# zhiqwang/demonet

Hardware: AMD Instinct MI355X
Metric: images/sec ssdlite320_mobilenet_v3_large fp16 end-to-end incl. NMS (higher is better)
Workload: dtype fp16; 1 GPU; ssdlite320_mobilenet_v3_large fp16, batch 64 per GPU, 320x320 synthetic images, K=91, synthetic weights seed 0, post-process incl. per-class top-300 + hard NMS; global_batch=64, forwards_in_flight=3, parallelism=single GPU, input=NCHW fp32 in [0,1], device-resident

## Files before the change

demonet_amd/_lib.py:

```python
import ctypes as C
import os

_HERE = os.path.dirname(os.path.abspath(__file__))
LIB_PATH = os.environ.get("DEMONET_HIP_LIB") or os.path.join(_HERE, "lib", "libdemonet_hip.so")
DN_ABI_VERSION = 1

DN_OP = dict(stem=1, pw=2, dw=3, se=4, conv=5, maxpool=6, l2norm=7)
DN_T = dict(act=0, image=1, vec=2, pool=3)
DN_NMS = dict(hard=0, linear=1, gaussian=2)
DN_MERGE = dict(iou=0, ios=1)
DN_SGD_CHUNK = 2048
DN_SGD_MAX_GATE = 8


class TensorDesc(C.Structure):
    _fields_ = [("c", C.c_int32), ("h", C.c_int32), ("w", C.c_int32), ("kind", C.c_int32)]


class OpDesc(C.Structure):
    _fields_ = [("type", C.c_int32), ("inp", C.c_int32), ("out", C.c_int32), ("residual", C.c_int32),
                ("se", C.c_int32), ("pool", C.c_int32),
                ("cin", C.c_int32), ("cout", C.c_int32), ("k", C.c_int32), ("stride", C.c_int32), ("pad", C.c_int32),
                ("dil", C.c_int32), ("act", C.c_int32),
                ("head", C.c_int32), ("level", C.c_int32), ("squeeze", C.c_int32), ("ceil_mode", C.c_int32),
                ("pool_pixels", C.c_int32), ("reserved", C.c_int32 * 2),
                ("w_off", C.c_int64), ("b_off", C.c_int64), ("w2_off", C.c_int64), ("b2_off", C.c_int64)]


class SgdTensor(C.Structure):
    _fields_ = [("p", C.c_void_p), ("g", C.c_void_p), ("buf", C.c_void_p), ("numel", C.c_int64)]


class SgdHyper(C.Structure):
    _fields_ = [("lr", C.c_float), ("momentum", C.c_float), ("dampening", C.c_float), ("weight_decay", C.c_float),
                ("nesterov", C.c_int32), ("first_step", C.c_int32), ("step", C.c_int32), ("reserved", C.c_int32)]


class ModelDesc(C.Structure):
    _fields_ = [("abi_version", C.c_int32), ("n_tensors", C.c_int32), ("n_ops", C.c_int32),
                ("tensors", C.POINTER(TensorDesc)), ("ops", C.POINTER(OpDesc)),
                ("input_tensor", C.c_int32), ("image_h", C.c_int32), ("image_w", C.c_int32),
                ("mean", C.c_float * 3), ("std", C.c_float * 3),
                ("num_classes", C.c_int32), ("n_levels", C.c_int32),
                ("level_tensor", C.c_int32 * 8), ("anchors_per_loc", C.c_int32 * 8),
                ("num_anchors", C.c_int32), ("anchors", C.POINTER(C.c_float)),
                ("score_thresh", C.c_float), ("nms_thresh", C.c_float),
                ("detections_per_img", C.c_int32), ("topk_candidates", C.c_int32)]


_SIGNATURES = {
    "dn_abi_version": (C.c_int, []),
    "dn_last_error": (C.c_char_p, []),
    "dn_create": (C.c_int, [C.POINTER(ModelDesc), C.c_void_p, C.c_size_t, C.POINTER(C.c_void_p)]),
    "dn_destroy": (None, [C.c_void_p]),
    "dn_workspace_bytes": (C.c_size_t, [C.c_void_p, C.c_int]),
    "dn_forward": (C.c_int, [C.c_void_p, C.c_void_p, C.c_int, C.c_int, C.c_int, C.c_void_p, C.c_void_p, C.c_void_p,
                             C.c_void_p, C.c_void_p, C.c_size_t, C.c_void_p]),
    "dn_forward_u8": (C.c_int, [C.c_void_p, C.c_void_p, C.c_int, C.c_int, C.c_int, C.c_void_p, C.c_void_p, C.c_void_p,
                             C.c_void_p, C.c_void_p, C.c_size_t, C.c_void_p]),
    "dn_forward_heads": (C.c_int, [C.c_void_p, C.c_void_p, C.c_int, C.c_int, C.c_int, C.c_void_p, C.c_size_t, C.c_void_p]),
    "dn_head_outputs": (C.c_int, [C.c_void_p, C.c_void_p, C.c_int, C.POINTER(C.c_void_p), C.POINTER(C.c_void_p)]),
    "dn_tensor_ptr": (C.c_int, [C.c_void_p, C.c_void_p, C.c_int, C.c_int, C.POINTER(C.c_void_p), C.POINTER(C.c_size_t)]),
    "dn_postprocess_workspace_bytes": (C.c_size_t, [C.c_int, C.c_int, C.c_int, C.c_int, C.c_int]),
    "dn_postprocess": (C.c_int, [C.c_void_p, C.c_void_p, C.c_void_p, C.c_int, C.c_int, C.c_int, C.c_float, C.c_float,
                                 C.c_void_p, C.c_float, C.c_float, C.c_int, C.c_int, C.c_void_p, C.c_void_p, C.c_void_p,
                                 C.c_void_p, C.c_void_p, C.c_void_p, C.c_size_t, C.c_void_p]),
    "dn_postprocess_soft": (C.c_int, [C.c_void_p, C.c_void_p, C.c_void_p, C.c_int, C.c_int, C.c_int, C.c_float, C.c_float,
                                      C.c_void_p, C.c_float, C.c_float, C.c_int, C.c_float, C.c_int, C.c_int, C.c_void_p, C.c_void_p, C.c_void_p,
                                      C.c_void_p, C.c_void_p, C.c_void_p, C.c_size_t, C.c_void_p]),
    "dn_set_nms": (C.c_int, [C.c_void_p, C.c_int, C.c_float]),
    "dn_pointwise_conv": (C.c_int, [C.c_void_p, C.c_void_p, C.c_void_p, C.c_void_p, C.c_void_p, C.c_void_p, C.c_void_p, C.c_int,
                                    C.c_int, C.c_int, C.c_int, C.c_int, C.c_int, C.c_int64, C.c_void_p]),
    "dn_depthwise_conv": (C.c_int, [C.c_void_p, C.c_void_p, C.c_void_p, C.c_void_p, C.c_int, C.c_int, C.c_int, C.c_int,
                                    C.c_int, C.c_int, C.c_int, C.c_int, C.c_void_p]),
    "dn_dense_conv": (C.c_int, [C.c_void_p] * 5 + [C.c_int] * 10 + [C.c_void_p]),
    "dn_expand_depthwise": (C.c_int, [C.c_void_p] * 9 + [C.c_int] * 11 + [C.c_void_p]),
    "dn_expand_depthwise_tiles": (C.c_int, [C.c_int, C.c_int, C.c_int]),
    "dn_ssd_loss_workspace_bytes": (C.c_size_t, [C.c_int, C.c_int]),
    "dn_ssd_loss": (C.c_int, [C.c_void_p] * 6 + [C.c_int] * 4 + [C.c_float, C.c_float] + [C.c_void_p, C.c_void_p, C.c_void_p, C.c_size_t, C.c_void_p]),
    "dn_ssd_loss_state_bytes": (C.c_size_t, [C.c_int, C.c_int]),
    "dn_ssd_loss_train": (C.c_int, [C.c_void_p] * 6 + [C.c_int] * 4 + [C.c_float, C.c_float] + [C.c_void_p, C.c_void_p, C.c_void_p, C.c_size_t, C.c_void_p, C.c_size_t,
                                    C.c_void_p]),
    "dn_ssd_loss_backward": (C.c_int, [C.c_void_p] * 6 + [C.c_size_t, C.c_void_p] + [C.c_int] * 4 + [C.c_void_p] * 3),
    "dn_set_graph_mode": (C.c_int, [C.c_void_p, C.c_int]),
    "dn_set_packed_output": (C.c_int, [C.c_void_p, C.c_void_p]),
    "dn_profile_begin": (C.c_int, [C.c_void_p]),
    "dn_profile_end": (C.c_int, [C.c_void_p, C.POINTER(C.c_float), C.c_int]),
    "dn_batch_split": (C.c_int, [C.c_void_p, C.c_int]),
    "dn_set_chains": (C.c_int, [C.c_void_p, C.c_int]),
    "dn_profile_op_info": (C.c_int, [C.c_void_p, C.c_int, C.c_char_p, C.c_int, C.POINTER(C.c_int32)]),
    "dn_level_features": (C.c_int, [C.c_void_p, C.c_void_p, C.c_int, C.c_int, C.c_int, C.POINTER(C.c_void_p), C.POINTER(C.c_int), C.POINTER(C.c_int)]),
    "dn_forward_features": (C.c_int, [C.c_void_p, C.c_void_p, C.c_int, C.c_int, C.c_int, C.c_void_p, C.c_size_t, C.c_void_p]),
    "dn_lite_head_backward_workspace_bytes": (C.c_size_t, [C.c_int] * 6),
    "dn_lite_head_backward": (C.c_int, [C.c_void_p] * 5 + [C.c_int64] + [C.c_int] * 5 + [C.c_void_p] * 5 + [C.c_size_t, C.c_void_p]),
    "dn_crop_tiles": (C.c_int, [C.c_void_p, C.c_int, C.c_int, C.c_void_p, C.c_int, C.c_int, C.c_int, C.c_void_p, C.c_void_p]),
    "dn_merge_detections_workspace_bytes": (C.c_size_t, [C.c_int] * 3),
    "dn_merge_detections": (C.c_int, [C.c_void_p] * 5 + [C.c_int, C.c_int, C.POINTER(C.c_int32), C.c_int, C.c_int, C.c_float, C.c_int, C.c_int] + [C.c_void_p] * 6
                            + [C.c_size_t, C.c_void_p]),
    "dn_fuse_detections_workspace_bytes": (C.c_size_t, [C.c_int, C.c_int, C.POINTER(C.c_int32), C.c_int]),
    "dn_fuse_detections": (C.c_int, [C.c_void_p] * 6 + [C.c_int, C.c_int, C.POINTER(C.c_int32), C.c_int, C.c_float, C.c_float, C.c_int] + [C.c_void_p] * 6
                           + [C.c_size_t, C.c_void_p]),
    "dn_match_detections": (C.c_int, [C.c_void_p] * 8 + [C.c_int] * 4 + [C.POINTER(C.c_double), C.c_int, C.c_double] + [C.c_void_p] * 5),
    "dn_coco_match": (C.c_int, [C.c_void_p] * 9 + [C.c_int] * 4 + [C.POINTER(C.c_double), C.c_int, C.POINTER(C.c_double), C.c_int, C.c_int] + [C.c_void_p] * 5),
    "dn_augment_workspace_bytes": (C.c_size_t, [C.c_int]),
    "dn_augment_batch": (C.c_int, [C.POINTER(C.c_void_p), C.POINTER(C.c_int32), C.POINTER(C.c_int32), C.c_int, C.c_int, C.c_int, C.c_void_p, C.c_void_p, C.c_size_t, C.c_void_p]),
    "dn_sgd_workspace_bytes": (C.c_size_t, [C.c_int, C.c_int]),
    "dn_grad_norm": (C.c_int, [C.c_void_p, C.c_int, C.c_int, C.c_void_p, C.c_size_t, C.c_void_p, C.c_void_p]),
    "dn_sgd_step": (C.c_int, [C.c_void_p, C.c_int, C.c_int, SgdHyper, C.c_void_p, C.c_int, C.c_void_p, C.c_float, C.c_void_p, C.c_void_p]),
}
EXPORTS = tuple(_SIGNATURES)

_lib = None


class HipLibraryMissing(RuntimeError):
    pass


def lib():
    global _lib
    if _lib is not None:
        return _lib
    if not os.path.exists(LIB_PATH):
        raise HipLibraryMissing(
            f"{LIB_PATH} not found: build it with `python -m demonet_amd.build` (hipcc, gfx950). "
            "demonet_amd has no CPU fallback.")
    L = C.CDLL(LIB_PATH)
    for name, (res, args) in _SIGNATURES.items():
        fn = getattr(L, name)
        fn.restype = res
        fn.argtypes = args
    if L.dn_abi_version() != DN_ABI_VERSION:
        raise HipLibraryMissing(f"ABI mismatch: library {L.dn_abi_version()} vs binding {DN_ABI_VERSION}; rebuild")
    _lib = L
    return L


def check(rc: int, what: str = ""):
    if rc < 0:
        msg = lib().dn_last_error().decode("utf-8", "replace")
        raise RuntimeError(f"demonet_hip {what} failed ({rc}): {msg}")
    return rc
```

demonet_amd/csrc/depthwise.hip:

```cpp
#include "choice.h"

#ifdef DN_DEV_STAMPS
static long long* g_se_stamps = nullptr;
extern "C" __attribute__((visibility("default"))) void dn_debug_se_stamps(void* dev_ptr) { g_se_stamps = (long long*)dev_ptr; }
#else
constexpr long long* g_se_stamps = nullptr;
#endif

namespace {

__device__ const uint4 g_dw_zero16 = {0u, 0u, 0u, 0u};

__device__ __forceinline__ void dw_se_tail(const DwArgs& a, const int n, const int nblk, float* sh) {
    const int c = a.c, sq = a.se_sq, tid = threadIdx.x;
    float* mean = sh;
    float* z = sh + c;
    float* part = z + sq;
    {
        const float* p0 = a.pool + (size_t)n * nblk * c;
        for (int ic = tid; ic < c; ic += 256) {
            float t = 0.f;
            for (int b0 = 0; b0 < nblk; b0 += 16) {
                float v[16];
#pragma unroll
                for (int u = 0; u < 16; ++u) v[u] = __hip_atomic_load(&p0[(size_t)min(b0 + u, nblk - 1) * c + ic], __ATOMIC_RELAXED, __HIP_MEMORY_SCOPE_AGENT);
#pragma unroll
                for (int u = 0; u < 16; ++u) t += (b0 + u < nblk) ? v[u] : 0.f;
            }
            mean[ic] = t * a.se_inv;
        }
    }
    __syncthreads();
    auto fc = [&](const half_t* wt, const float* bias, const float* in, int nin, int nout, float* out, bool hsig) {
        const int OG = (nout + 7) >> 3;
        int ogp = 1;
        while (ogp < OG) ogp <<= 1;
        const int KS = 256 / ogp;
        const int og = tid & (ogp - 1), ks = tid / ogp;
        const int per = (nin + KS - 1) / KS, i0 = ks * per, i1 = min(nin, i0 + per);
        float acc[8] = {0, 0, 0, 0, 0, 0, 0, 0};
        if (og < OG && i0 < i1) {
            const half_t* wp = wt + (size_t)og * 8;
            for (int ib = i0; ib < i1; ib += 16) {
                uint4 v[16];
#pragma unroll
                for (int u = 0; u < 16; ++u) v[u] = *reinterpret_cast<const uint4*>(wp + (size_t)min(ib + u, i1 - 1) * nout);
#pragma unroll
                for (int u = 0; u < 16; ++u) {
                    const float m = (ib + u < i1) ? in[ib + u] : 0.f;
                    const half8 h = *reinterpret_cast<const half8*>(&v[u]);
#pragma unroll
                    for (int e = 0; e < 8; ++e) acc[e] += (float)h[e] * m;
                }
            }
        }
#pragma unroll
        for (int e = 0; e < 8; ++e) part[tid * 8 + e] = acc[e];
        __syncthreads();
        for (int j = tid; j < nout; j += 256) {
            float t = bias[j];
            const int g = j >> 3, e = j & 7;
            for (int q = 0; q < KS; ++q) t += part[(q * ogp + g) * 8 + e];
            out[j] = hsig ? fminf(fmaxf(t + 3.f, 0.f), 6.f) * (1.f / 6.f) : fmaxf(t, 0.f);
        }
        __syncthreads();
    };
    fc(a.se_w1t, a.se_b1, mean, c, sq, z, false);
    fc(a.se_w2t, a.se_b2, z, sq, c, a.se_scale + (size_t)n * c, true);
}

__device__ __forceinline__ void dw_se_tail_small(const DwArgs& a, const int n, const int nblk, float* sh) {
    const int c = a.c, sq = a.se_sq, tid = threadIdx.x;
    float* mean = sh;
    float* z = sh + c;
    float* part = z + sq;
    const int OG1 = (sq + 7) >> 3, OG2 = (c + 7) >> 3;
    int ogp1 = 1, ogp2 = 1;
    while (ogp1 < OG1) ogp1 <<= 1;
    while (ogp2 < OG2) ogp2 <<= 1;
    const int KS1 = 256 / ogp1, KS2 = 256 / ogp2;
    const int og1 = tid & (ogp1 - 1), ks1 = tid / ogp1, per1 = (c + KS1 - 1) / KS1, i0 = ks1 * per1, i1 = min(c, i0 + per1);
    const int og2 = tid & (ogp2 - 1), ks2 = tid / ogp2, per2 = (sq + KS2 - 1) / KS2, j0 = ks2 * per2, j1 = min(sq, j0 + per2);
    const bool act1 = og1 < OG1 && i0 < i1, act2 = og2 < OG2 && j0 < j1;
    float pv[32];
    {
        const float* p0 = a.pool + (size_t)n * nblk * c + min(tid, c - 1);
#pragma unroll
        for (int b = 0; b < 32; ++b) pv[b] = __hip_atomic_load(&p0[(size_t)min(b, nblk - 1) * c], __ATOMIC_RELAXED, __HIP_MEMORY_SCOPE_AGENT);
    }
    uint4 w1[2], w2[2];
#pragma unroll
    for (int u = 0; u < 2; ++u) {
        w1[u] = *reinterpret_cast<const uint4*>(a.se_w1t + (size_t)min(i0 + u, c - 1) * sq + min(og1, OG1 - 1) * 8);
        w2[u] = *reinterpret_cast<const uint4*>(a.se_w2t + (size_t)min(j0 + u, sq - 1) * c + min(og2, OG2 - 1) * 8);
    }
    const float b1v = a.se_b1[min(tid, sq - 1)], b2v = a.se_b2[min(tid, c - 1)];
    if (tid < c) {
        float t = 0.f;
#pragma unroll
        for (int b = 0; b < 32; ++b) t += (b < nblk) ? pv[b] : 0.f;
        mean[tid] = t * a.se_inv;
    }
    __syncthreads();
    auto fc = [&](const uint4 (&w)[2], bool act, int r0, int r1, const float* in, int ogp, int KS, int nout, float bias, float* out, bool hsig) {
        float acc[8] = {0, 0, 0, 0, 0, 0, 0, 0};
        if (act) {
#pragma unroll
            for (int u = 0; u < 2; ++u) {
                const float m = (r0 + u < r1) ? in[r0 + u] : 0.f;
                const half8 h = *reinterpret_cast<const half8*>(&w[u]);
#pragma unroll
                for (int e = 0; e < 8; ++e) acc[e] += (float)h[e] * m;
            }
        }
#pragma unroll
        for (int e = 0; e < 8; ++e) part[tid * 8 + e] = acc[e];
        __syncthreads();
        if (tid < nout) {
            float t = bias;
            const int g = tid >> 3, e = tid & 7;
            for (int q = 0; q < KS; ++q) t += part[(q * ogp + g) * 8 + e];
            out[tid] = hsig ? fminf(fmaxf(t + 3.f, 0.f), 6.f) * (1.f / 6.f) : fmaxf(t, 0.f);
        }
        __syncthreads();
    };
    fc(w1, act1, i0, i1, mean, ogp1, KS1, sq, b1v, z, false);
    fc(w2, act2, j0, j1, z, ogp2, KS2, c, b2v, a.se_scale + (size_t)n * c, true);
}
__device__ __forceinline__ bool dw_se_tail_is_small(int c, int sq, int nblk) {
    if (!(se_is_small(c, sq) && nblk <= 32)) return false;
    int ogp1 = 1, ogp2 = 1;
    while (ogp1 < ((sq + 7) >> 3)) ogp1 <<= 1;
    while (ogp2 < ((c + 7) >> 3)) ogp2 <<= 1;
    const int ks1 = 256 / ogp1, ks2 = 256 / ogp2;
    return (c + ks1 - 1) / ks1 <= 2 && (sq + ks2 - 1) / ks2 <= 2;
}

template <int K, int S, int TW, int POOL>
__device__ __forceinline__ void dw_body(const DwArgs& a, const int bx, const int nblocks, const int n) {
    constexpr int NIN = (TW - 1) * S + K;
    extern __shared__ float red[];
    const unsigned C8 = a.c >> 3;
    const unsigned idx0 = bx * 256 + threadIdx.x;
    const unsigned q1 = fd_div(idx0, a.fd_c8);
    const unsigned cg = idx0 - q1 * C8;
    const unsigned oy = fd_div(q1, a.fd_xs);
    const unsigned xs = q1 - oy * a.fd_xs.d;
    const bool valid = (int)oy < a.ho;
    if (!valid && POOL == 0) return;
    const int ox0 = xs * TW;
    const unsigned c0 = cg * 8;
    float psum[8] = {0, 0, 0, 0, 0, 0, 0, 0};
    if (valid) {

    float acc[TW][8];
    {
        const float4 b0 = *reinterpret_cast<const float4*>(a.bias + c0);
        const float4 b1 = *reinterpret_cast<const float4*>(a.bias + c0 + 4);
#pragma unroll
        for (int t = 0; t < TW; ++t) {
            acc[t][0] = b0.x; acc[t][1] = b0.y; acc[t][2] = b0.z; acc[t][3] = b0.w;
            acc[t][4] = b1.x; acc[t][5] = b1.y; acc[t][6] = b1.z; acc[t][7] = b1.w;
        }
    }
    const int ix0 = ox0 * S - a.pad;
    typedef const __attribute__((address_space(1))) half8* gp8;
    const gp8 zero = (gp8)(&g_dw_zero16);
    const half_t* const wbase = a.w + c0;
    const half_t* const xbase = a.x + (size_t)n * a.h * a.w_ * a.c + c0;
    half8 wv[2][K];
    half8 xin[2][NIN];
    auto load_row = [&](const int ky, const int buf) {
        const int iy = (int)oy * S - a.pad + ky;
        const bool yok = iy >= 0 && iy < a.h;
#pragma unroll
        for (int kx = 0; kx < K; ++kx) wv[buf][kx] = *reinterpret_cast<const half8*>(wbase + (unsigned)((ky * K + kx) * a.c));
        const half_t* rowp = xbase + (unsigned)((yok ? iy : 0) * a.w_ * a.c);
#pragma unroll
        for (int i = 0; i < NIN; ++i) {
            const int ix = ix0 + i;
            const bool ok = yok && ix >= 0 && ix < a.w_;
            xin[buf][i] = *(ok ? (gp8)(rowp + (unsigned)(ix * a.c)) : zero);
        }
    };
    load_row(0, 0);
#pragma unroll
    for (int ky = 0; ky < K; ++ky) {
        if (ky + 1 < K) load_row(ky + 1, (ky + 1) & 1);
#pragma unroll
        for (int t = 0; t < TW; ++t)
#pragma unroll
            for (int kx = 0; kx < K; ++kx)
                fma_mix_h8(acc[t], *reinterpret_cast<const uint4*>(&xin[ky & 1][t * S + kx]), *reinterpret_cast<const uint4*>(&wv[ky & 1][kx]));
    }
    half_t* orow = a.out + ((size_t)(n * a.ho + oy) * a.wo) * a.c + c0;
#pragma unroll
    for (int t = 0; t < TW; ++t) {
        if (ox0 + t >= a.wo) break;
        dn_act_n<float[8], 8>(acc[t], a.act);
        half8 o;
#pragma unroll
        for (int e = 0; e < 8; ++e) {
            if constexpr (POOL != 0) psum[e] += acc[t][e];
            o[e] = (half_t)acc[t][e];
        }
        *reinterpret_cast<half8*>(orow + (unsigned)((ox0 + t) * a.c)) = o;
    }
    }
    if constexpr (POOL != 0) {
#pragma unroll
        for (int e = 0; e < 8; ++e) red[threadIdx.x * 8 + e] = psum[e];
        __syncthreads();
        if (threadIdx.x < C8) {
            const unsigned i1 = bx * 256 + threadIdx.x;
            const unsigned cgp = i1 - fd_div(i1, a.fd_c8) * C8;
            float t8[8] = {0, 0, 0, 0, 0, 0, 0, 0};
            for (unsigned u = threadIdx.x; u < 256; u += C8)
#pragma unroll
                for (int e = 0; e < 8; ++e) t8[e] += red[u * 8 + e];
            float* dst = a.pool + ((size_t)n * nblocks + bx) * a.c + cgp * 8;
            if constexpr (POOL == 2) {
#pragma unroll
                for (int e = 0; e < 8; ++e) __hip_atomic_store(&dst[e], t8[e], __ATOMIC_RELAXED, __HIP_MEMORY_SCOPE_AGENT);
                asm volatile("s_waitcnt vmcnt(0)" ::: "memory");
            } else {
#pragma unroll
                for (int e = 0; e < 8; ++e) dst[e] = t8[e];
            }
        }
        if constexpr (POOL == 2) {
            __shared__ int s_last;
            __syncthreads();
            if (threadIdx.x == 0)
                s_last = __hip_atomic_fetch_add(&a.se_counter[n], 1u, __ATOMIC_RELAXED, __HIP_MEMORY_SCOPE_AGENT) == (unsigned)(nblocks - 1);
            __syncthreads();
            if (s_last) {
                if (dw_se_tail_is_small(a.c, a.se_sq, nblocks)) dw_se_tail_small(a, n, nblocks, red);
                else dw_se_tail(a, n, nblocks, red);
                if (threadIdx.x == 0) a.se_counter[n] = 0u;
            }
        }
    }
}

template <int K, int S, int TW, int POOL>
__global__ __launch_bounds__(256) __attribute__((amdgpu_waves_per_eu(K == 3 ? 4 : 3))) void dw_kernel(DwArgs a, int nblocks) {
    int img, bx;
    if (!xcd_image_of2(a.xq, a.n, img, bx)) return;
    dw_body<K, S, TW, POOL>(a, bx, nblocks, img);
}

struct DwGroup {
    int count;
    int start[13];
    int nblocks[12];
    DwArgs a[12];
};

template <int K, int S, int TW>
__global__ __launch_bounds__(256) __attribute__((amdgpu_waves_per_eu(K == 3 ? 4 : 1))) void dw_group_kernel(DwGroup g) {
    int p = 0;
#pragma unroll
    for (int i = 1; i < 12; ++i)
        if (i < g.count && (int)blockIdx.x >= g.start[i]) p = i;
    const DwArgs& a = g.a[p];
    const int rel = blockIdx.x - g.start[p];
    int img, bx;
    if (a.xq > 0) { img = (rel & 7) * a.xq + blockIdx.y; bx = rel >> 3; }
    else { img = blockIdx.y; bx = rel; }
    if (img >= a.n) return;
    dw_body<K, S, TW, 0>(a, bx, g.nblocks[p], img);
}

bool dw_fill(DwArgs& a, const int tw) {
    const unsigned c8 = a.c / 8, xs = (a.wo + tw - 1) / tw;
    a.fd_c8 = fastdiv(c8);
    a.fd_xs = fastdiv(xs);
    const unsigned long long threads = (unsigned long long)a.ho * xs * c8 + 256;
    return fd_ok(threads, c8) && fd_ok(threads / c8 + 1, xs) && (unsigned long long)a.h * a.w_ * a.c < 0x80000000ull;
}
int dw_blocks(const DwArgs& a, const int tw) { return dn_cdiv((long)a.ho * ((a.wo + tw - 1) / tw) * (a.c / 8), 256); }

template <int K_, int S_>
struct DwInst { static constexpr int K = K_, S = S_, TW = dw_tw(S_); };
template <class F>
int dw_dispatch(const DwChoice& c, F&& f) {
    if (c.k == 3 && c.stride == 1) return f(DwInst<3, 1>{});
    if (c.k == 3 && c.stride == 2) return f(DwInst<3, 2>{});
    if (c.k == 5 && c.stride == 1) return f(DwInst<5, 1>{});
    if (c.k == 5 && c.stride == 2) return f(DwInst<5, 2>{});
    dn_set_error("depthwise: unsupported k=%d stride=%d", c.k, c.stride);
    return DN_E_UNSUPPORTED;
}

template <int K, int S, int TW>
int launch_dw_group(const DwArgs* arr, int count, hipStream_t s) {
    DwGroup g{};
    g.count = count;
    int acc = 0;
    for (int i = 0; i < count; ++i) {
        g.a[i] = arr[i];
        DN_REQUIRE(dw_fill(g.a[i], TW), "depthwise group: problem %d outside the index range of the kernel", i);
        g.start[i] = acc;
        g.nblocks[i] = dw_blocks(arr[i], TW);
        acc += g.nblocks[i] * (arr[i].xq > 0 ? 8 : 1);
    }
    g.start[count] = acc;
    dn_note_kernel("dw_group_kernel<%d,%d,%d>", K, S, TW);
    hipLaunchKernelGGL((dw_group_kernel<K, S, TW>), dim3(acc, arr[0].xq > 0 ? arr[0].xq : arr[0].n), dim3(256), 0, s, g);
    return DN_OK;
}

template <int K, int S, int TW>
int launch_dw(const DwArgs& a0, const DwChoice::Pool pool, hipStream_t s) {
    DwArgs a = a0;
    DN_REQUIRE(dw_fill(a, TW), "depthwise: %d x %d x %d outside the index range of the kernel", a.ho, a.wo, a.c);
    dn_note_kernel("dw_kernel<%d,%d,%d>", K, S, TW);
    const int nblocks = dw_blocks(a, TW);
    const dim3 grid = xcd_grid2(nblocks, a.xq, a.n);
    switch (pool) {
        case DwChoice::NO_POOL: hipLaunchKernelGGL((dw_kernel<K, S, TW, 0>), grid, dim3(256), 0, s, a, nblocks); break;
        case DwChoice::POOLED: hipLaunchKernelGGL((dw_kernel<K, S, TW, 1>), grid, dim3(256), (size_t)256 * 8 * 4, s, a, nblocks); break;
        case DwChoice::POOLED_SE:
            DN_REQUIRE(a.pool && a.se_counter && depthwise_se_tail_supported(a.c, a.se_sq), "depthwise: squeeze-excitation tail needs the pooled output and c <= 1024, squeeze <= 256, both multiples of 8");
            hipLaunchKernelGGL((dw_kernel<K, S, TW, 2>), grid, dim3(256), (size_t)(a.c + a.se_sq + 2048) * 4, s, a, nblocks);
            break;
    }
    return DN_OK;
}

__global__ __launch_bounds__(1024) void se_fc_kernel(const float* __restrict__ partial, int nblk, const unsigned* __restrict__ w1t,
                                                   const float* __restrict__ b1, const unsigned* __restrict__ w2t,
                                                   const float* __restrict__ b2, float* __restrict__ scale,
                                                   int c, int sq, float inv_pixels, long long* __restrict__ stamps, int nimg, int xq) {
#ifdef DN_DEV_STAMPS
#define SE_STAMP(k) do { if (stamps && threadIdx.x == 0) stamps[blockIdx.x * 8 + (k)] = (long long)__builtin_amdgcn_s_memrealtime(); } while (0)
#else
#define SE_STAMP(k) do { } while (0)
#endif
    extern __shared__ float sh[];
    float* mean = sh;
    float* z = sh + c;
    float* part = z + sq;
    int n, unused;
    if (!xcd_image_of(blockIdx.x, 1, xq, nimg, n, unused)) return;
    const int tid = threadIdx.x;
    SE_STAMP(0);
    const int sq2 = sq >> 1, c2 = c >> 1;
    const int JP = sq2;
    const int KS1 = 1024 / JP;
    const int j = tid % JP, r1 = tid / JP;
    const int per1 = (c + KS1 - 1) / KS1;
    const int i0 = r1 * per1, i1 = min(c, i0 + per1);
    const bool act1 = j < sq2 && r1 < KS1;
    const int CP = c2;
    const int KS2 = max(1, 1024 / CP);
    const int i = tid % CP, r2 = tid / CP;
    const int per2 = (sq + KS2 - 1) / KS2;
    const int j0 = r2 * per2, j1 = min(sq, j0 + per2);
    const bool act2 = i < c2 && r2 < KS2;
    constexpr int FB = 32;
    {
        const int CPm = (c + 63) & ~63;
        const int RS = max(1, min(1024 / CPm, nblk));
        const int ic = tid % CPm, r = tid / CPm;
        float t = 0.f;
        if (ic < c && r < RS) {
            const float* p = partial + (size_t)n * nblk * c + ic;
            for (int b0 = r; b0 < nblk; b0 += RS * 16) {
                float v[16];
#pragma unroll
                for (int u = 0; u < 16; ++u) v[u] = p[(size_t)min(b0 + u * RS, nblk - 1) * c];
#pragma unroll
                for (int u = 0; u < 16; ++u) t += (b0 + u * RS < nblk) ? v[u] : 0.f;
            }
        }
        part[tid] = t;
        __syncthreads();
        if (tid < c) {
            float m = 0.f;
            for (int q = 0; q < RS; ++q) m += part[q * CPm + tid];
            mean[tid] = m * inv_pixels;
        }
        __syncthreads();
    }
    SE_STAMP(1);
    auto lo = [](unsigned w) { return (float)__builtin_bit_cast(half_t, (unsigned short)(w & 0xffffu)); };
    auto hi = [](unsigned w) { return (float)__builtin_bit_cast(half_t, (unsigned short)(w >> 16)); };
    {
        float t0 = 0.f, t1 = 0.f;
        if (act1) {
            for (int ib = i0; ib < i1; ib += FB) {
                unsigned v[FB];
#pragma unroll
                for (int u = 0; u < FB; ++u) v[u] = w1t[(size_t)min(ib + u, i1 - 1) * sq2 + j];
#pragma unroll
                for (int u = 0; u < FB; ++u) {
                    const float m = (ib + u < i1) ? mean[ib + u] : 0.f;
                    t0 += lo(v[u]) * m;
                    t1 += hi(v[u]) * m;
                }
            }
        }
        part[tid] = t0;
        part[1024 + tid] = t1;
        __syncthreads();
        if (tid < sq) {
            float a = b1[tid];
// ... 773 lines not shown
```

demonet_amd/csrc/plan.hip:

```cpp
#include <stdarg.h>
#include <stdlib.h>
#include <string.h>

#include <algorithm>
#include <cmath>
#include <atomic>
#include <map>
#include <mutex>
#include <set>
#include <string>
#include <tuple>
#include <vector>

#include "choice.h"

static thread_local char g_err[512] = "";

static thread_local char g_kernel[96] = "";
void dn_note_kernel(const char* fmt, ...) {
    va_list ap;
    va_start(ap, fmt);
    vsnprintf(g_kernel, sizeof(g_kernel), fmt, ap);
    va_end(ap);
}
// ... 1342 lines not shown
    return launch_postprocess(a, reinterpret_cast<hipStream_t>(stream), nullptr);
}

extern "C" int dn_postprocess(const float* logits, const float* reg, const float* anchors, int n, int A, int K, float image_h,
                              float image_w, const float* scale_xy, float score_thresh, float nms_thresh, int topk, int dets,
                              float* boxes, float* scores, int64_t* labels, int32_t* counts, int32_t* kept_anchor, void* ws,
                              size_t ws_bytes, void* stream) {
    return dn_postprocess_soft(logits, reg, anchors, n, A, K, image_h, image_w, scale_xy, score_thresh, nms_thresh, DN_NMS_HARD, 0.f, topk, dets,
                               boxes, scores, labels, counts, kept_anchor, ws, ws_bytes, stream);
}

extern "C" int dn_pointwise_conv(const void* x, const void* w, const void* w_frag, const float* bias, const void* residual,
                                 const float* se, void* out, int m, int cin, int cout, int hw, int act, int out_fp32,
                                 int64_t out_img_stride, void* stream) {
    DN_REQUIRE(x && w && bias && out, "dn_pointwise_conv: null argument");
    PwArgs a;
    a.x = reinterpret_cast<const half_t*>(x); a.w = reinterpret_cast<const half_t*>(w); a.bias = bias;
    a.wfrag = reinterpret_cast<const half_t*>(w_frag);
    a.residual = reinterpret_cast<const half_t*>(residual); a.se = se; a.out = out;
    a.m = m; a.cin = cin; a.cout = cout; a.hw = hw; a.act = act; a.out_fp32 = out_fp32;
    a.out_img_stride = out_fp32 ? (long)out_img_stride : 0; a.out_base = 0;
    a.xq = (hw > 0 && m % hw == 0) ? xcd_images_per_group(m / hw) : 0;
    int rc = launch_pointwise(a, reinterpret_cast<hipStream_t>(stream));
    if (rc) return rc;
    DN_HIP_CHECK(hipGetLastError());
    return DN_OK;
}

extern "C" int dn_expand_depthwise(const void* x, const void* w1, const float* b1, const void* wd, const float* bd, const void* w3,
                                   const float* b3, void* out, float* pool_partial, int n, int h, int w, int cin, int cexp, int cout,
                                   int k, int stride, int act1, int act2, int has_res, void* stream) {
    DN_REQUIRE(x && wd && bd && out, "dn_expand_depthwise: null argument");
    DN_REQUIRE((w1 == nullptr) == (b1 == nullptr) && (w3 == nullptr) == (b3 == nullptr), "dn_expand_depthwise: weight without bias");
    ExpDwArgs a{};
    a.x = reinterpret_cast<const half_t*>(x); a.out = reinterpret_cast<half_t*>(out); a.pool = pool_partial;
    a.w1 = reinterpret_cast<const half_t*>(w1); a.b1 = b1; a.wd = reinterpret_cast<const half_t*>(wd); a.bd = bd;
    a.w3 = reinterpret_cast<const half_t*>(w3); a.b3 = b3;
    a.n = n; a.H = h; a.W = w; a.k = k; a.stride = stride; a.pad = (k - 1) / 2;
    a.Ho = (h + 2 * a.pad - k) / stride + 1; a.Wo = (w + 2 * a.pad - k) / stride + 1;
    a.cin = cin; a.cexp = cexp; a.cout = w3 ? cout : cexp; a.act1 = act1; a.act2 = act2; a.has_res = has_res;
    a.xq = xcd_images_per_group(n);
    int rc = launch_expdw(a, reinterpret_cast<hipStream_t>(stream));
    if (rc) return rc;
    DN_HIP_CHECK(hipGetLastError());
    return DN_OK;
}

extern "C" int dn_expand_depthwise_tiles(int ho, int wo, int stride) { return expdw_tiles_per_image(ho, wo, stride); }

extern "C" int dn_dense_conv(const void* x, const void* w, const float* bias, const void* zeros, void* out, int n, int h, int wd,
                             int cin, int cout, int k, int stride, int pad, int dil, int act, void* stream) {
    DN_REQUIRE(x && w && bias && out, "dn_dense_conv: null argument");
    DN_REQUIRE(n > 0 && h > 0 && wd > 0 && k >= 1 && stride >= 1 && dil >= 1 && pad >= 0, "dn_dense_conv: bad geometry");
    ConvArgs a;
    a.x = reinterpret_cast<const half_t*>(x); a.w = reinterpret_cast<const half_t*>(w); a.bias = bias; a.out = out;
    a.zeros = reinterpret_cast<const half_t*>(zeros);
    a.n = n; a.h = h; a.w_ = wd; a.cin = cin; a.cout = cout; a.k = k; a.stride = stride; a.pad = pad; a.dil = dil; a.act = act;
    a.ho = (h + 2 * pad - dil * (k - 1) - 1) / stride + 1;
    a.wo = (wd + 2 * pad - dil * (k - 1) - 1) / stride + 1;
    DN_REQUIRE(a.ho > 0 && a.wo > 0, "dn_dense_conv: empty output");
    a.out_fp32 = 0; a.out_img_stride = 0; a.out_base = 0;
    a.xq = xcd_images_per_group(n);
    int rc = launch_conv(a, reinterpret_cast<hipStream_t>(stream));
    if (rc) return rc;
    DN_HIP_CHECK(hipGetLastError());
    return DN_OK;
}

extern "C" int dn_depthwise_conv(const void* x, const void* w, const float* bias, void* out, int n, int h, int wd, int c, int k,
                                 int stride, int pad, int act, void* stream) {
    DN_REQUIRE(x && w && bias && out, "dn_depthwise_conv: null argument");
    DwArgs a;
    a.x = reinterpret_cast<const half_t*>(x); a.w = reinterpret_cast<const half_t*>(w); a.bias = bias;
    a.out = reinterpret_cast<half_t*>(out);
    a.n = n; a.h = h; a.w_ = wd; a.c = c; a.k = k; a.stride = stride; a.pad = pad; a.act = act;
    a.ho = (h + 2 * pad - k) / stride + 1;
    a.wo = (wd + 2 * pad - k) / stride + 1;
    a.xq = xcd_images_per_group(n);
    int rc = launch_depthwise(a, reinterpret_cast<hipStream_t>(stream));
    if (rc) return rc;
    DN_HIP_CHECK(hipGetLastError());
    return DN_OK;
}
```

include/demonet_hip.h:

```cpp
#ifndef DEMONET_HIP_H
#define DEMONET_HIP_H

#include <stddef.h>
#include <stdint.h>

#ifdef __cplusplus
extern "C" {
#endif

#define DN_ABI_VERSION 1
#define DN_MAX_CLASSES 2048
#define DN_API __attribute__((visibility("default")))

enum { DN_OK = 0, DN_E_INVALID = -1, DN_E_HIP = -2, DN_E_WORKSPACE = -3, DN_E_UNSUPPORTED = -4 };

enum { DN_ACT_NONE = 0, DN_ACT_RELU = 1, DN_ACT_RELU6 = 2, DN_ACT_HSWISH = 3 };

enum { DN_OP_STEM = 1, DN_OP_PW = 2, DN_OP_DW = 3, DN_OP_SE = 4, DN_OP_CONV = 5, DN_OP_MAXPOOL = 6, DN_OP_L2NORM = 7 };

enum { DN_T_ACT = 0, DN_T_IMAGE = 1, DN_T_VEC = 2, DN_T_POOL = 3 };

typedef struct dn_tensor_desc {
    int32_t c, h, w, kind;
} dn_tensor_desc;

typedef struct dn_op_desc {
    int32_t type;
    int32_t in, out;
    int32_t residual;
    int32_t se;
    int32_t pool;
    int32_t cin, cout, k, stride, pad, dil, act;
    int32_t head;
    int32_t level;
    int32_t squeeze;
    int32_t ceil_mode;
    int32_t pool_pixels;
    int32_t reserved[2];
    int64_t w_off, b_off, w2_off, b2_off;
} dn_op_desc;

typedef struct dn_model_desc {
    int32_t abi_version;
    int32_t n_tensors, n_ops;
    const dn_tensor_desc* tensors;
    const dn_op_desc* ops;
    int32_t input_tensor;
    int32_t image_h, image_w;
    float mean[3], std[3];
    int32_t num_classes;
    int32_t n_levels;
    int32_t level_tensor[8];
    int32_t anchors_per_loc[8];
    int32_t num_anchors;
    const float* anchors;
    float score_thresh, nms_thresh;
    int32_t detections_per_img, topk_candidates;
} dn_model_desc;

typedef struct dn_plan dn_plan;

DN_API int dn_create(const dn_model_desc* desc, const void* weights, size_t weight_bytes, dn_plan** out);
DN_API void dn_destroy(dn_plan* plan);

DN_API size_t dn_workspace_bytes(const dn_plan* plan, int n);

DN_API int dn_forward(dn_plan* plan, const float* images_dev, int n, int h, int w,
               float* boxes_dev, float* scores_dev, int64_t* labels_dev, int32_t* counts_dev,
               void* workspace_dev, size_t workspace_bytes, void* stream);

DN_API int dn_forward_u8(dn_plan* plan, const uint8_t* images_dev, int n, int h, int w,
                  float* boxes_dev, float* scores_dev, int64_t* labels_dev, int32_t* counts_dev,
                  void* workspace_dev, size_t workspace_bytes, void* stream);

DN_API int dn_forward_heads(dn_plan* plan, const float* images_dev, int n, int h, int w,
                     void* workspace_dev, size_t workspace_bytes, void* stream);
DN_API int dn_head_outputs(const dn_plan* plan, void* workspace_dev, int n, float** cls_logits_dev, float** bbox_regression_dev);
DN_API int dn_tensor_ptr(const dn_plan* plan, void* workspace_dev, int n, int tensor_id, void** ptr, size_t* bytes);

DN_API int dn_level_features(const dn_plan* plan, void* workspace_dev, int n, int level, int chain, void** ptr, int* first_image, int* images);
DN_API int dn_forward_features(dn_plan* plan, const float* images_dev, int n, int h, int w,
                               void* workspace_dev, size_t workspace_bytes, void* stream);

DN_API size_t dn_postprocess_workspace_bytes(int n, int num_anchors, int num_classes, int topk_candidates, int detections_per_img);
DN_API int dn_postprocess(const float* cls_logits_dev, const float* bbox_regression_dev, const float* anchors_dev,
                   int n, int num_anchors, int num_classes,
                   float image_h, float image_w, const float* scale_xy_dev ,
                   float score_thresh, float nms_thresh, int topk_candidates, int detections_per_img,
                   float* boxes_dev, float* scores_dev, int64_t* labels_dev, int32_t* counts_dev,
                   int32_t* kept_anchor_dev, void* workspace_dev, size_t workspace_bytes, void* stream);

enum { DN_NMS_HARD = 0, DN_NMS_SOFT_LINEAR = 1, DN_NMS_SOFT_GAUSSIAN = 2 };
DN_API int dn_set_nms(dn_plan* plan, int method, float sigma);
DN_API int dn_postprocess_soft(const float* cls_logits_dev, const float* bbox_regression_dev, const float* anchors_dev,
                   int n, int num_anchors, int num_classes,
                   float image_h, float image_w, const float* scale_xy_dev ,
                   float score_thresh, float nms_thresh, int nms_method, float nms_sigma, int topk_candidates, int detections_per_img,
                   float* boxes_dev, float* scores_dev, int64_t* labels_dev, int32_t* counts_dev,
                   int32_t* kept_anchor_dev, void* workspace_dev, size_t workspace_bytes, void* stream);

DN_API int dn_pointwise_conv(const void* x_dev, const void* w_dev, const void* w_frag_dev, const float* bias_dev,
                      const void* residual_dev, const float* se_scale_dev, void* out_dev, int m, int cin, int cout, int hw,
                      int act, int out_fp32, int64_t out_img_stride, void* stream);
DN_API int dn_dense_conv(const void* x_dev, const void* w_dev, const float* bias_dev, const void* zeros_dev, void* out_dev,
                  int n, int h, int w, int cin, int cout, int k, int stride, int pad, int dil, int act, void* stream);
DN_API int dn_depthwise_conv(const void* x_dev, const void* w_dev, const float* bias_dev, void* out_dev,
                      int n, int h, int w, int c, int k, int stride, int pad, int act, void* stream);

DN_API int dn_expand_depthwise(const void* x_dev, const void* w1_dev, const float* b1_dev, const void* wd_dev, const float* bd_dev,
                        const void* w3_dev, const float* b3_dev, void* out_dev, float* pool_partial_dev,
                        int n, int h, int w, int cin, int cexp, int cout, int k, int stride, int act1, int act2, int has_res,
                        void* stream);
DN_API int dn_expand_depthwise_tiles(int ho, int wo, int stride);

DN_API int dn_set_graph_mode(dn_plan* plan, int enabled);

DN_API int dn_profile_begin(dn_plan* plan);
DN_API int dn_profile_end(dn_plan* plan, float* ms_per_op , int capacity);
DN_API int dn_profile_op_info(const dn_plan* plan, int op_index, char* kernel, int capacity, int32_t* owner);

DN_API int dn_set_packed_output(dn_plan* plan, float* packed_dev);

DN_API int dn_batch_split(const dn_plan* plan, int n);
DN_API int dn_set_chains(dn_plan* plan, int chains);

DN_API size_t dn_ssd_loss_workspace_bytes(int n, int num_anchors);
DN_API int dn_ssd_loss(const float* cls_logits_dev, const float* bbox_regression_dev, const float* anchors_dev,
                       const float* gt_boxes_dev, const int64_t* gt_labels_dev, const int32_t* gt_counts_dev,
                       int n, int num_anchors, int num_classes, int gmax, float iou_thresh, float neg_to_pos_ratio,
                       int64_t* matched_idxs_dev, float* losses_dev, void* workspace_dev, size_t workspace_bytes, void* stream);

DN_API size_t dn_ssd_loss_state_bytes(int n, int num_anchors);
DN_API int dn_ssd_loss_train(const float* cls_logits_dev, const float* bbox_regression_dev, const float* anchors_dev,
                             const float* gt_boxes_dev, const int64_t* gt_labels_dev, const int32_t* gt_counts_dev,
                             int n, int num_anchors, int num_classes, int gmax, float iou_thresh, float neg_to_pos_ratio,
                             int64_t* matched_idxs_dev, float* losses_dev, void* workspace_dev, size_t workspace_bytes,
                             void* state_dev, size_t state_bytes, void* stream);
DN_API int dn_ssd_loss_backward(const float* cls_logits_dev, const float* bbox_regression_dev, const float* anchors_dev,
                                const float* gt_boxes_dev, const int64_t* gt_labels_dev, const void* state_dev, size_t state_bytes,
                                const float* grad_losses_dev, int n, int num_anchors, int num_classes, int gmax,
                                float* grad_cls_logits_dev, float* grad_bbox_regression_dev, void* stream);

DN_API size_t dn_lite_head_backward_workspace_bytes(int n, int h, int w, int c, int cout, int depthwise);
DN_API int dn_lite_head_backward(const void* x_dev, const void* wd_dev, const float* bd_dev, const void* w1_dev, const float* dy_dev,
                                 int64_t dy_img_stride, int n, int h, int w, int c, int cout, float* g_wd_dev, float* g_bd_dev,
                                 float* g_w1_dev, float* g_b1_dev, void* workspace_dev, size_t workspace_bytes, void* stream);

DN_API int dn_crop_tiles(const float* image_dev, int h, int w, const int32_t* origins_dev, int t, int th, int tw, float* out_dev, void* stream);

enum { DN_MERGE_IOU = 0, DN_MERGE_IOS = 1 };
DN_API size_t dn_merge_detections_workspace_bytes(int s_total, int d, int groups);
DN_API int dn_merge_detections(const float* boxes_dev, const float* scores_dev, const int64_t* labels_dev, const int32_t* counts_dev,
                               const float* offsets_dev, int s_total, int d, const int32_t* group_begin, int groups, int metric, float thresh,
                               int class_agnostic, int d_out, float* boxes_out_dev, float* scores_out_dev, int64_t* labels_out_dev,
                               int32_t* counts_out_dev, int32_t* src_out_dev, void* workspace_dev, size_t workspace_bytes, void* stream);

DN_API size_t dn_fuse_detections_workspace_bytes(int s_total, int d, const int32_t* group_begin, int groups);
DN_API int dn_fuse_detections(const float* boxes_dev, const float* scores_dev, const int64_t* labels_dev, const int32_t* counts_dev,
                              const float* offsets_dev, const float* weights_dev, int s_total, int d, const int32_t* group_begin, int groups,
                              float thresh, float skip_thresh, int d_out, float* boxes_out_dev, float* scores_out_dev, int64_t* labels_out_dev,
                              int32_t* counts_out_dev, int32_t* members_out_dev, void* workspace_dev, size_t workspace_bytes, void* stream);

DN_API int dn_match_detections(const float* boxes_dev, const float* scores_dev, const int64_t* labels_dev, const int32_t* counts_dev,
                               const float* gt_boxes_dev, const int64_t* gt_labels_dev, const uint8_t* gt_difficult_dev,
                               const int32_t* gt_counts_dev, int n, int d, int gmax, int num_classes, const double* thresholds, int n_thresh,
                               double pixel_offset, uint32_t* flags_dev, int32_t* best_gt_dev, double* best_ov_dev, int64_t* gt_stats_dev,
                               void* stream);

DN_API int dn_coco_match(const float* boxes_dev, const float* scores_dev, const int64_t* labels_dev, const int32_t* counts_dev,
                         const float* gt_boxes_dev, const int64_t* gt_labels_dev, const int32_t* gt_counts_dev, const uint8_t* gt_crowd_dev,
                         const float* gt_area_dev, int n, int d, int gmax, int num_classes, const double* thresholds, int n_thresh,
                         const double* area_ranges, int n_ranges, int max_det, uint32_t* flags_dev, int32_t* rank_dev, int32_t* match_gt_dev,
                         int64_t* gt_stats_dev, void* stream);

enum { DN_AUG_FLAGS = 0,
       DN_AUG_BRIGHTNESS = 1, DN_AUG_CONTRAST = 2, DN_AUG_SATURATION = 3, DN_AUG_HUE = 4,
       DN_AUG_PERM = 5,
       DN_AUG_CANVAS_H = 8, DN_AUG_CANVAS_W = 9, DN_AUG_LEFT = 10, DN_AUG_TOP = 11,
       DN_AUG_FILL = 12,
       DN_AUG_CROP_L = 15, DN_AUG_CROP_T = 16, DN_AUG_CROP_W = 17, DN_AUG_CROP_H = 18,
       DN_AUG_WORDS = 20 };
enum { DN_AUG_F_BRIGHTNESS = 1, DN_AUG_F_CONTRAST = 2, DN_AUG_F_SATURATION = 4, DN_AUG_F_HUE = 8, DN_AUG_F_CONTRAST_BEFORE = 16, DN_AUG_F_FLIP = 32,
       DN_AUG_F_ALL = 63 };
DN_API size_t dn_augment_workspace_bytes(int n);
DN_API int dn_augment_batch(const uint8_t* const* images, const int32_t* sizes, const int32_t* params, int n, int out_h, int out_w,
                            float* out_dev, void* workspace_dev, size_t workspace_bytes, void* stream);

#define DN_SGD_CHUNK 2048
#define DN_SGD_MAX_GATE 8
typedef struct dn_sgd_tensor {
// ... 24 lines not shown
```

Baseline: 107,300 images/sec.

## Stage depthwise weights and bias in LDS and use buffer loads for inputs

For depthwise convolutions with at most 128 channels, each block now copies the filter taps (transposed so each channel group's taps are contiguous) and the bias into shared memory, then reads weights from LDS instead of global memory. Input rows are fetched with raw buffer loads whose out-of-range offsets return zero, replacing the pointer select to a zero constant. The first input row is prefetched before the weight staging to overlap the two. It also adds a pooled depthwise API entry point and debug timestamp hooks. The cost is extra shared memory per block and a block-wide barrier, which may reduce occupancy; the waves-per-EU hint is raised for this path.

```diff
diff --git a/demonet_amd/_lib.py b/demonet_amd/_lib.py
--- a/demonet_amd/_lib.py
+++ b/demonet_amd/_lib.py
@@ -73,6 +73,8 @@
                                     C.c_int, C.c_int, C.c_int, C.c_int, C.c_int, C.c_int64, C.c_void_p]),
     "dn_depthwise_conv": (C.c_int, [C.c_void_p, C.c_void_p, C.c_void_p, C.c_void_p, C.c_int, C.c_int, C.c_int, C.c_int,
                                     C.c_int, C.c_int, C.c_int, C.c_int, C.c_void_p]),
+    "dn_depthwise_pool_blocks": (C.c_int, [C.c_int] * 6),
+    "dn_depthwise_conv_pool": (C.c_int, [C.c_void_p] * 4 + [C.c_int] * 8 + [C.c_void_p] * 7 + [C.c_int, C.c_void_p]),
     "dn_dense_conv": (C.c_int, [C.c_void_p] * 5 + [C.c_int] * 10 + [C.c_void_p]),
     "dn_expand_depthwise": (C.c_int, [C.c_void_p] * 9 + [C.c_int] * 11 + [C.c_void_p]),
     "dn_expand_depthwise_tiles": (C.c_int, [C.c_int, C.c_int, C.c_int]),
diff --git a/demonet_amd/csrc/depthwise.hip b/demonet_amd/csrc/depthwise.hip
--- a/demonet_amd/csrc/depthwise.hip
+++ b/demonet_amd/csrc/depthwise.hip
@@ -3,8 +3,16 @@
 #ifdef DN_DEV_STAMPS
 static long long* g_se_stamps = nullptr;
 extern "C" __attribute__((visibility("default"))) void dn_debug_se_stamps(void* dev_ptr) { g_se_stamps = (long long*)dev_ptr; }
+static long long* g_dw_stamps = nullptr;
+extern "C" __attribute__((visibility("default"))) void dn_debug_dw_stamps(void* dev_ptr) { g_dw_stamps = (long long*)dev_ptr; }
+#define DW_STAMPS_PARAM , long long* const stamps
+#define DW_STAMPS_ARG(p) , p
+#define DW_STAMP(k) do { if (stamps && threadIdx.x == 0) stamps[((size_t)n * nblocks + bx) * 8 + (k)] = (long long)__builtin_amdgcn_s_memrealtime(); } while (0)
 #else
 constexpr long long* g_se_stamps = nullptr;
+#define DW_STAMPS_PARAM
+#define DW_STAMPS_ARG(p)
+#define DW_STAMP(k) do { } while (0)
 #endif
 
 namespace {
@@ -136,10 +144,12 @@
     return (c + ks1 - 1) / ks1 <= 2 && (sq + ks2 - 1) / ks2 <= 2;
 }
 
-template <int K, int S, int TW, int POOL>
-__device__ __forceinline__ void dw_body(const DwArgs& a, const int bx, const int nblocks, const int n) {
-    constexpr int NIN = (TW - 1) * S + K;
-    extern __shared__ float red[];
+template <int K, int S, int TW, int POOL, bool WLDS>
+__device__ __forceinline__ void dw_body(const DwArgs& a, const int bx, const int nblocks, const int n DW_STAMPS_PARAM) {
+    constexpr int NIN = (TW - 1) * S + K, KK = K * K;
+    extern __shared__ __attribute__((aligned(16))) float dw_sh[];
+    float* const red = WLDS ? dw_sh + (KK * a.c) / 2 + a.c : dw_sh;
+    DW_STAMP(0);
     const unsigned C8 = a.c >> 3;
     const unsigned idx0 = bx * 256 + threadIdx.x;
     const unsigned q1 = fd_div(idx0, a.fd_c8);
@@ -147,30 +157,66 @@
     const unsigned oy = fd_div(q1, a.fd_xs);
     const unsigned xs = q1 - oy * a.fd_xs.d;
     const bool valid = (int)oy < a.ho;
-    if (!valid && POOL == 0) return;
+    if (!valid && POOL == 0 && !WLDS) return;
     const int ox0 = xs * TW;
     const unsigned c0 = cg * 8;
+    const int ix0 = ox0 * S - a.pad;
     float psum[8] = {0, 0, 0, 0, 0, 0, 0, 0};
+    half8 xin[2][NIN];
+    const unsigned c2 = (unsigned)a.c * 2u;
+    const __amdgpu_buffer_rsrc_t xrs = __builtin_amdgcn_make_buffer_rsrc(const_cast<half_t*>(a.x + (size_t)n * a.h * a.w_ * a.c), 0, WLDS ? a.h * a.w_ * a.c * 2 : 0, 0x00020000);
+    auto load_row_buf = [&](const int ky, const int buf) {
+        const int iy = (int)oy * S - a.pad + ky;
+        const bool yok = valid && (unsigned)iy < (unsigned)a.h;
+        const unsigned rowoff = (unsigned)((iy * a.w_ + ix0) * a.c + (int)c0) * 2u;
+#pragma unroll
+        for (int i = 0; i < NIN; ++i) {
+            const bool ok = yok && (unsigned)(ix0 + i) < (unsigned)a.w_;
+            xin[buf][i] = __builtin_bit_cast(half8, __builtin_amdgcn_raw_buffer_load_b128(xrs, ok ? rowoff + (unsigned)i * c2 : 0x80000000u, 0, 0));
+        }
+    };
+    if constexpr (WLDS) {
+        load_row_buf(0, 0);
+        const uint4* const wsrc = reinterpret_cast<const uint4*>(a.w);
+        uint4* const wdst = reinterpret_cast<uint4*>(dw_sh);
+        const unsigned nitems = KK * C8;
+        const unsigned one = a.fd_c8.d == 1 ? ~0u : 0u;
+        float4* const bdst = reinterpret_cast<float4*>(dw_sh + (KK * a.c) / 2);
+        const unsigned bi = min(threadIdx.x, ((unsigned)a.c >> 2) - 1);
+        const float4 bv = reinterpret_cast<const float4*>(a.bias)[bi];
+        for (unsigned i0 = threadIdx.x; i0 < nitems; i0 += 1024) {
+            uint4 v[4];
+#pragma unroll
+            for (int u = 0; u < 4; ++u) v[u] = wsrc[min(i0 + u * 256, nitems - 1)];
+#pragma unroll
+            for (int u = 0; u < 4; ++u) {
+                const unsigned i = min(i0 + u * 256, nitems - 1), tap = __umulhi(i, a.fd_c8.m) + (i & one);
+                wdst[(i - tap * C8) * KK + tap] = v[u];
+            }
+        }
+        bdst[bi] = bv;
+        __syncthreads();
+    }
+    DW_STAMP(1);
     if (valid) {
 
     float acc[TW][8];
     {
-        const float4 b0 = *reinterpret_cast<const float4*>(a.bias + c0);
-        const float4 b1 = *reinterpret_cast<const float4*>(a.bias + c0 + 4);
+        const float* const bsrc = WLDS ? dw_sh + (KK * a.c) / 2 : a.bias;
+        const float4 b0 = *reinterpret_cast<const float4*>(bsrc + c0);
+        const float4 b1 = *reinterpret_cast<const float4*>(bsrc + c0 + 4);
 #pragma unroll
         for (int t = 0; t < TW; ++t) {
             acc[t][0] = b0.x; acc[t][1] = b0.y; acc[t][2] = b0.z; acc[t][3] = b0.w;
             acc[t][4] = b1.x; acc[t][5] = b1.y; acc[t][6] = b1.z; acc[t][7] = b1.w;
         }
     }
-    const int ix0 = ox0 * S - a.pad;
     typedef const __attribute__((address_space(1))) half8* gp8;
     const gp8 zero = (gp8)(&g_dw_zero16);
     const half_t* const wbase = a.w + c0;
     const half_t* const xbase = a.x + (size_t)n * a.h * a.w_ * a.c + c0;
     half8 wv[2][K];
-    half8 xin[2][NIN];
-    auto load_row = [&](const int ky, const int buf) {
+    auto load_row_ptr = [&](const int ky, const int buf) {
         const int iy = (int)oy * S - a.pad + ky;
         const bool yok = iy >= 0 && iy < a.h;
 #pragma unroll
@@ -183,20 +229,42 @@
             xin[buf][i] = *(ok ? (gp8)(rowp + (unsigned)(ix * a.c)) : zero);
         }
     };
-    load_row(0, 0);
+    auto load_row = [&](const int ky, const int buf) {
+        if constexpr (WLDS) load_row_buf(ky, buf);
+        else load_row_ptr(ky, buf);
+    };
+    const uint4* const wl = reinterpret_cast<const uint4*>(dw_sh) + cg * KK;
+    if constexpr (!WLDS) load_row(0, 0);
 #pragma unroll
     for (int ky = 0; ky < K; ++ky) {
         if (ky + 1 < K) load_row(ky + 1, (ky + 1) & 1);
-#pragma unroll
-        for (int t = 0; t < TW; ++t)
-#pragma unroll
-            for (int kx = 0; kx < K; ++kx)
-                fma_mix_h8(acc[t], *reinterpret_cast<const uint4*>(&xin[ky & 1][t * S + kx]), *reinterpret_cast<const uint4*>(&wv[ky & 1][kx]));
-    }
+        if constexpr (WLDS) {
+#pragma unroll
+            for (int kx = 0; kx < K; ++kx) {
+                const uint4 w = wl[ky * K + kx];
+#pragma unroll
+                for (int t = 0; t < TW; ++t) fma_mix_h8(acc[t], *reinterpret_cast<const uint4*>(&xin[ky & 1][t * S + kx]), w);
+            }
+        } else {
+#pragma unroll
+            for (int t = 0; t < TW; ++t)
+#pragma unroll
+                for (int kx = 0; kx < K; ++kx)
+                    fma_mix_h8(acc[t], *reinterpret_cast<const uint4*>(&xin[ky & 1][t * S + kx]), *reinterpret_cast<const uint4*>(&wv[ky & 1][kx]));
+        }
+    }
+    DW_STAMP(2);
     half_t* orow = a.out + ((size_t)(n * a.ho + oy) * a.wo) * a.c + c0;
+    int ox0s = ox0;
+    if constexpr (POOL != 0 && !WLDS) {
+        unsigned t2 = threadIdx.x;
+        asm volatile("" : "+v"(t2));
+        const unsigned q2 = fd_div(bx * 256 + t2, a.fd_c8);
+        ox0s = (int)(q2 - fd_div(q2, a.fd_xs) * a.fd_xs.d) * TW;
+    }
 #pragma unroll
     for (int t = 0; t < TW; ++t) {
-        if (ox0 + t >= a.wo) break;
+        if (ox0s + t >= a.wo) break;
         dn_act_n<float[8], 8>(acc[t], a.act);
         half8 o;
 #pragma unroll
@@ -204,9 +272,10 @@
             if constexpr (POOL != 0) psum[e] += acc[t][e];
             o[e] = (half_t)acc[t][e];
         }
-        *reinterpret_cast<half8*>(orow + (unsigned)((ox0 + t) * a.c)) = o;
-    }
-    }
+        *reinterpret_cast<half8*>(orow + (unsigned)((ox0s + t) * a.c)) = o;
+    }
+    }
+    DW_STAMP(3);
     if constexpr (POOL != 0) {
 #pragma unroll
         for (int e = 0; e < 8; ++e) red[threadIdx.x * 8 + e] = psum[e];
@@ -230,24 +299,27 @@
         }
         if constexpr (POOL == 2) {
             __shared__ int s_last;
+            DW_STAMP(4);
             __syncthreads();
             if (threadIdx.x == 0)
                 s_last = __hip_atomic_fetch_add(&a.se_counter[n], 1u, __ATOMIC_RELAXED, __HIP_MEMORY_SCOPE_AGENT) == (unsigned)(nblocks - 1);
             __syncthreads();
+            DW_STAMP(5);
             if (s_last) {
-                if (dw_se_tail_is_small(a.c, a.se_sq, nblocks)) dw_se_tail_small(a, n, nblocks, red);
-                else dw_se_tail(a, n, nblocks, red);
+                if (dw_se_tail_is_small(a.c, a.se_sq, nblocks)) dw_se_tail_small(a, n, nblocks, dw_sh);
+                else dw_se_tail(a, n, nblocks, dw_sh);
                 if (threadIdx.x == 0) a.se_counter[n] = 0u;
-            }
-        }
-    }
-}
-
-template <int K, int S, int TW, int POOL>
-__global__ __launch_bounds__(256) __attribute__((amdgpu_waves_per_eu(K == 3 ? 4 : 3))) void dw_kernel(DwArgs a, int nblocks) {
+                DW_STAMP(6);
+            }
+        }
+    }
+}
+
+template <int K, int S, int TW, int POOL, bool WLDS>
+__global__ __launch_bounds__(256) __attribute__((amdgpu_waves_per_eu(K == 3 || WLDS ? 4 : 3))) void dw_kernel(DwArgs a, int nblocks DW_STAMPS_PARAM) {
     int img, bx;
     if (!xcd_image_of2(a.xq, a.n, img, bx)) return;
-    dw_body<K, S, TW, POOL>(a, bx, nblocks, img);
+    dw_body<K, S, TW, POOL, WLDS>(a, bx, nblocks, img DW_STAMPS_ARG(stamps));
 }
 
 struct DwGroup {
@@ -269,7 +341,7 @@
     if (a.xq > 0) { img = (rel & 7) * a.xq + blockIdx.y; bx = rel >> 3; }
     else { img = blockIdx.y; bx = rel; }
     if (img >= a.n) return;
-    dw_body<K, S, TW, 0>(a, bx, g.nblocks[p], img);
+    dw_body<K, S, TW, 0, false>(a, bx, g.nblocks[p], img DW_STAMPS_ARG(nullptr));
 }
 
 bool dw_fill(DwArgs& a, const int tw) {
@@ -280,6 +352,14 @@
     return fd_ok(threads, c8) && fd_ok(threads / c8 + 1, xs) && (unsigned long long)a.h * a.w_ * a.c < 0x80000000ull;
 }
 int dw_blocks(const DwArgs& a, const int tw) { return dn_cdiv((long)a.ho * ((a.wo + tw - 1) / tw) * (a.c / 8), 256); }
+
+size_t dw_wlds_bytes(const DwArgs& a, const int k) {
+    const int knob = dn_knob("DN_DW_WLDS", 1);
+    if (knob == 0 || (knob != 2 && a.c > 128)) return 0;
+    const size_t bytes = (size_t)k * k * a.c * 2 + (size_t)a.c * 4;
+    const bool ok = a.c <= 1024 && bytes + 256 * 8 * 4 <= 64 * 1024 && (unsigned long long)a.h * a.w_ * a.c < 0x40000000ull && fd_ok((unsigned long long)k * k * (a.c / 8) + 1024, a.c / 8);
+    return ok ? bytes : 0;
+}
 
 template <int K_, int S_>
 struct DwInst { static constexpr int K = K_, S = S_, TW = dw_tw(S_); };
@@ -318,12 +398,21 @@
     dn_note_kernel("dw_kernel<%d,%d,%d>", K, S, TW);
     const int nblocks = dw_blocks(a, TW);
     const dim3 grid = xcd_grid2(nblocks, a.xq, a.n);
+    const size_t red = (size_t)256 * 8 * 4, tail = (size_t)(a.c + a.se_sq + 2048) * 4;
+    const size_t wl = dw_wlds_bytes(a, K);
     switch (pool) {
-        case DwChoice::NO_POOL: hipLaunchKernelGGL((dw_kernel<K, S, TW, 0>), grid, dim3(256), 0, s, a, nblocks); break;
-        case DwChoice::POOLED: hipLaunchKernelGGL((dw_kernel<K, S, TW, 1>), grid, dim3(256), (size_t)256 * 8 * 4, s, a, nblocks); break;
+        case DwChoice::NO_POOL:
+            if (wl) hipLaunchKernelGGL((dw_kernel<K, S, TW, 0, true>), grid, dim3(256), wl, s, a, nblocks DW_STAMPS_ARG(g_dw_stamps));
+            else hipLaunchKernelGGL((dw_kernel<K, S, TW, 0, false>), grid, dim3(256), 0, s, a, nblocks DW_STAMPS_ARG(g_dw_stamps));
+            break;
+        case DwChoice::POOLED:
+            if (wl) hipLaunchKernelGGL((dw_kernel<K, S, TW, 1, true>), grid, dim3(256), wl + red, s, a, nblocks DW_STAMPS_ARG(g_dw_stamps));
+            else hipLaunchKernelGGL((dw_kernel<K, S, TW, 1, false>), grid, dim3(256), red, s, a, nblocks DW_STAMPS_ARG(g_dw_stamps));
+            break;
         case DwChoice::POOLED_SE:
             DN_REQUIRE(a.pool && a.se_counter && depthwise_se_tail_supported(a.c, a.se_sq), "depthwise: squeeze-excitation tail needs the pooled output and c <= 1024, squeeze <= 256, both multiples of 8");
-            hipLaunchKernelGGL((dw_kernel<K, S, TW, 2>), grid, dim3(256), (size_t)(a.c + a.se_sq + 2048) * 4, s, a, nblocks);
+            if (wl) hipLaunchKernelGGL((dw_kernel<K, S, TW, 2, true>), grid, dim3(256), std::max(wl + red, tail), s, a, nblocks DW_STAMPS_ARG(g_dw_stamps));
+            else hipLaunchKernelGGL((dw_kernel<K, S, TW, 2, false>), grid, dim3(256), tail, s, a, nblocks DW_STAMPS_ARG(g_dw_stamps));
             break;
     }
     return DN_OK;
diff --git a/demonet_amd/csrc/plan.hip b/demonet_amd/csrc/plan.hip
--- a/demonet_amd/csrc/plan.hip
+++ b/demonet_amd/csrc/plan.hip
@@ -1448,3 +1448,36 @@
     DN_HIP_CHECK(hipGetLastError());
     return DN_OK;
 }
+
+extern "C" int dn_depthwise_pool_blocks(int h, int wd, int c, int k, int stride, int pad) {
+    DwArgs a{};
+    a.n = 1; a.h = h; a.w_ = wd; a.c = c; a.k = k; a.stride = stride; a.pad = pad;
+    a.ho = (h + 2 * pad - k) / stride + 1;
+    a.wo = (wd + 2 * pad - k) / stride + 1;
+    return depthwise_pool_blocks(a);
+}
+
+extern "C" int dn_depthwise_conv_pool(const void* x, const void* w, const float* bias, void* out, int n, int h, int wd, int c, int k,
+                                      int stride, int pad, int act, float* pool, const void* se_w1t, const float* se_b1, const void* se_w2t,
+                                      const float* se_b2, float* se_scale, unsigned* se_counter, int squeeze, void* stream) {
+    DN_REQUIRE(x && w && bias && out && pool, "dn_depthwise_conv_pool: null argument");
+    DN_REQUIRE(!se_scale || (se_w1t && se_b1 && se_w2t && se_b2 && se_counter), "dn_depthwise_conv_pool: the squeeze-excitation tail needs both FCs and the counters");
+    DwArgs a;
+    a.x = reinterpret_cast<const half_t*>(x); a.w = reinterpret_cast<const half_t*>(w); a.bias = bias;
+    a.out = reinterpret_cast<half_t*>(out);
+    a.n = n; a.h = h; a.w_ = wd; a.c = c; a.k = k; a.stride = stride; a.pad = pad; a.act = act;
+    a.ho = (h + 2 * pad - k) / stride + 1;
+    a.wo = (wd + 2 * pad - k) / stride + 1;
+    a.xq = xcd_images_per_group(n);
+    a.pool = pool;
+    if (se_scale) {
+        a.se_w1t = reinterpret_cast<const half_t*>(se_w1t); a.se_b1 = se_b1;
+        a.se_w2t = reinterpret_cast<const half_t*>(se_w2t); a.se_b2 = se_b2;
+        a.se_scale = se_scale; a.se_counter = se_counter; a.se_sq = squeeze;
+        a.se_inv = 1.0f / (float)(a.ho * a.wo);
+    }
+    int rc = launch_depthwise(a, reinterpret_cast<hipStream_t>(stream));
+    if (rc) return rc;
+    DN_HIP_CHECK(hipGetLastError());
+    return DN_OK;
+}
diff --git a/include/demonet_hip.h b/include/demonet_hip.h
--- a/include/demonet_hip.h
+++ b/include/demonet_hip.h
@@ -106,6 +106,11 @@
                   int n, int h, int w, int cin, int cout, int k, int stride, int pad, int dil, int act, void* stream);
 DN_API int dn_depthwise_conv(const void* x_dev, const void* w_dev, const float* bias_dev, void* out_dev,
                       int n, int h, int w, int c, int k, int stride, int pad, int act, void* stream);
+DN_API int dn_depthwise_pool_blocks(int h, int w, int c, int k, int stride, int pad);
+DN_API int dn_depthwise_conv_pool(const void* x_dev, const void* w_dev, const float* bias_dev, void* out_dev,
+                      int n, int h, int w, int c, int k, int stride, int pad, int act, float* pool_dev,
+                      const void* se_w1t_dev, const float* se_b1_dev, const void* se_w2t_dev, const float* se_b2_dev,
+                      float* se_scale_dev, unsigned* se_counter_dev, int squeeze, void* stream);
 
 DN_API int dn_expand_depthwise(const void* x_dev, const void* w1_dev, const float* b1_dev, const void* wd_dev, const float* bd_dev,
                         const void* w3_dev, const float* b3_dev, void* out_dev, float* pool_partial_dev,
```

New measurement: 109,500 images/sec, median of 6. 2.0% higher.
